# ZhehuiWu/MP-HSIR

Hardware: AMD Instinct MI355X
Metric: hsi_patches_per_sec_fwd_bwd (higher is better)
Workload: dtype bf16; 1 GPU; natural-scene MP_HSIR_Net(31,31,64,T=6) training step fwd+bwd+allreduce+AdamW, 64x64x31 patches, batch 32/GPU, dp1; global_batch=32, patch=64x64x31, parallelism=dp1, launch=hipGraph replay

## Files before the change

include/mphsir.h:

```cpp
#ifndef MPHSIR_H
#define MPHSIR_H
#include <stddef.h>
#include <stdint.h>

#ifdef __cplusplus
extern "C" {
#endif

#define MPHSIR_OK 0
#define MPHSIR_EINVAL (-1)
#define MPHSIR_ELAUNCH (-2)

#define MPHSIR_F32 0
#define MPHSIR_BF16 1
#define MPHSIR_F16 2

const char* mphsir_version(void);
const char* mphsir_last_error(void);
int mphsir_device_arch(char* buf, int n);

typedef struct mphsir_gemm_args {
    uint32_t struct_size;
    const void* X; int64_t ldx;
    const void* W; int64_t w_batch_stride; int64_t rows_per_batch;
// ... 129 lines not shown
    const void* W1; const float* b1; const void* W1T; const void* W2T;
    void* dX; void* XN; void* H; void* DPRE; float* part;
    int64_t M; int32_t C, HP;
    int32_t variant;
    const float* keep;
    int64_t rows_per_batch;
    int32_t hsplit;
    float* dxn_part;
} mphsir_mlp_bwd_args;
int mphsir_gated_mlp_bwd(const mphsir_mlp_bwd_args* a, int dtype, void* stream);

typedef struct mphsir_mlp_wgrad_args {
    uint32_t struct_size;
    const void* XN; const void* DM;
    const void* W1; const float* b1; const void* W2T;
    float* dW1p; float* dW2p; float* db1p; float* db2p;
    int64_t M; int32_t C, HP;
    int32_t ranges;
    int32_t chunks_per_wg;
} mphsir_mlp_wgrad_args;
int mphsir_gated_mlp_wgrad(const mphsir_mlp_wgrad_args* a, int dtype, void* stream);
int mphsir_gated_mlp_wgrad_fits(int32_t C, int32_t chunks_per_wg, int dtype);

int mphsir_combine_bwd(const void* dY, const void* SA, const float* gate, const float* keep, void* dOut, void* dSA,
                       float* dgate, int32_t B, int32_t H, int32_t W, int32_t C, int32_t shift, int dtype, void* stream);
typedef struct mphsir_win_attn_bwd_args {
    uint32_t struct_size;
    const void* X; const void* dSA; const float* dmu;
    const float* ln_w; const float* ln_b;
    const void* Wqkv; const float* bqkv; const float* rpb; const void* WprojT;
    void* dQKV; void* XNw; void* dSAt; float* drpb;
    int32_t B, H, W, C, heads, shift;
    int32_t head_split;
} mphsir_win_attn_bwd_args;
int mphsir_win_attn_bwd(const mphsir_win_attn_bwd_args* a, int dtype, void* stream);
int mphsir_win_attn_bwd_fits(int32_t C, int32_t heads, int dtype);
int mphsir_ln_bwd_win(const void* X, const void* dXNw, const void* dRes, const float* ln_w, void* dX, float* part,
                      int32_t B, int32_t H, int32_t W, int32_t C, int32_t shift, const float* ln_b, void* XN, int32_t linear,
                      int dtype, void* stream);

int mphsir_ln_bwd_win_dxn(const void* X, const void* dQKV, const void* WqkvT, const void* dRes, const void* dRes2, const float* ln_w, void* dX,
                          float* part, int32_t B, int32_t H, int32_t W, int32_t C, int32_t shift, int dtype, void* stream);
int mphsir_ln_bwd_win_dxn_fits(int32_t C, int dtype);
int mphsir_ln_bwd_tok_dxn(const void* X, const void* dY, const void* WT, const void* dRes, const float* ln_w, const float* ln_b, void* dX,
                          void* XN, float* part, int64_t M, int32_t C, int32_t K, int32_t x_f32, int dtype, void* stream);

int mphsir_layernorm_tok(const void* X, int x_dtype, const float* ln_w, const float* ln_b, void* Y, void* Xcopy, int y_dtype,
                         int64_t M, int32_t C, void* stream);

typedef struct mphsir_fold_bwd_args {
    uint32_t struct_size;
    const float* Gpart; const float* Spart; const float* temperature; const float* Wo; const float* dM;
    void* W2; float* dWo; float* dtemp;
    int32_t B, C, heads, nsplit;
    int32_t dM_nsplit;
    const void* DO; int64_t lddo; const void* V; int64_t ldv; int32_t N;
    int32_t w2_blocks;
} mphsir_fold_bwd_args;
int mphsir_spectral_fold_bwd(const mphsir_fold_bwd_args* a, int dtype, void* stream);
typedef struct mphsir_pg_bwd_args {
    uint32_t struct_size;
    const float* mu; const float* dgate;
    const float* Wprompt; const float* prompt_param; const float* Wq; const float* Wkv; const float* Wdown;
    const float* Wpproj; const float* bpproj; const float* Wup;
    float* dmu; void* L; void* R;
    int32_t nW, C, r, KL, KR;
    int32_t lr_bf16;
} mphsir_pg_bwd_args;
int mphsir_pg_gate_bwd(const mphsir_pg_bwd_args* a, void* stream);
// ... 241 lines not shown
```

mp-hsir_amd/_lib.py:

```python
import ctypes
import os

import torch

_HERE = os.path.dirname(os.path.abspath(__file__))
_PATH = os.path.join(_HERE, os.environ.get("MPHSIR_LIB_AB", "libmphsir.so"))
_lib = None
_is_emu = False

c_void_p, c_int64, c_int32, c_int, c_float_p = (ctypes.c_void_p, ctypes.c_int64, ctypes.c_int32, ctypes.c_int,
                                                ctypes.POINTER(ctypes.c_float))


class _Args(ctypes.Structure):

    def __init__(self, *args, **kw):
        super().__init__(*args, **kw)
        self.struct_size = ctypes.sizeof(self)


_SZ = [("struct_size", ctypes.c_uint32)]


class GemmArgs(_Args):
# ... 37 lines not shown
               [("T", c_void_p), ("ldt", c_int64), ("QK", c_void_p), ("ldqk", c_int64), ("row_segments", c_int32)]


class FoldArgs(_Args):
    _fields_ = _SZ + [("Gpart", c_void_p), ("Spart", c_void_p), ("temperature", c_void_p), ("Wo", c_void_p), ("M", c_void_p),
                ("MT", c_void_p)] + \
               [(n, c_int32) for n in ("B", "C", "heads", "nsplit")] + [("Gsum", c_void_p), ("Ssum", c_void_p)]


class GateArgs(_Args):
    _fields_ = _SZ + [("T", c_void_p), ("ldt", c_int64), ("w9", c_void_p), ("ldw", c_int64), ("U", c_void_p), ("ldu", c_int64)] + \
               [(n, c_int32) for n in ("B", "H", "W", "HP")]


class GdfnArgs(_Args):
    _fields_ = _SZ + [("X", c_void_p), ("ldx", c_int64), ("ln_w", c_void_p), ("ln_b", c_void_p), ("Win", c_void_p), ("w9", c_void_p),
                ("ldw", c_int64), ("Wout", c_void_p), ("Y", c_void_p), ("ldy", c_int64)] + \
               [(n, c_int32) for n in ("B", "H", "W", "D", "HP", "nsplit")] + [("T", c_void_p), ("ldt", c_int64)]


class MlpBwdArgs(_Args):
    _fields_ = _SZ + [(n, c_void_p) for n in ("X", "dY", "DM", "ln_w", "ln_b", "W1", "b1", "W1T", "W2T", "dX", "XN", "H", "DPRE", "part")] + \
               [("M", c_int64), ("C", c_int32), ("HP", c_int32), ("variant", c_int32), ("keep", c_void_p), ("rows_per_batch", c_int64),
                ("hsplit", c_int32), ("dxn_part", c_void_p)]


class MlpWgradArgs(_Args):
    _fields_ = _SZ + [(n, c_void_p) for n in ("XN", "DM", "W1", "b1", "W2T", "dW1p", "dW2p", "db1p", "db2p")] + \
               [("M", c_int64), ("C", c_int32), ("HP", c_int32), ("ranges", c_int32), ("chunks_per_wg", c_int32)]


class WinAttnBwdArgs(_Args):
    _fields_ = _SZ + [(n, c_void_p) for n in ("X", "dSA", "dmu", "ln_w", "ln_b", "Wqkv", "bqkv", "rpb", "WprojT", "dQKV", "XNw",
                                         "dSAt", "drpb")] + [(n, c_int32) for n in ("B", "H", "W", "C", "heads", "shift", "head_split")]


class FoldBwdArgs(_Args):
    _fields_ = _SZ + [(n, c_void_p) for n in ("Gpart", "Spart", "temperature", "Wo", "dM", "W2", "dWo", "dtemp")] + \
               [(n, c_int32) for n in ("B", "C", "heads", "nsplit", "dM_nsplit")] + \
               [("DO", c_void_p), ("lddo", c_int64), ("V", c_void_p), ("ldv", c_int64), ("N", c_int32), ("w2_blocks", c_int32)]


class PgBwdArgs(_Args):
    _fields_ = _SZ + [(n, c_void_p) for n in ("mu", "dgate", "Wprompt", "prompt_param", "Wq", "Wkv", "Wdown", "Wpproj", "bpproj", "Wup",
                                         "dmu", "L", "R")] + [(n, c_int32) for n in ("nW", "C", "r", "KL", "KR", "lr_bf16")]


class SpectralBwdArgs(_Args):
    _fields_ = _SZ + [("QK", c_void_p), ("ldqk", c_int64), ("DO", c_void_p), ("lddo", c_int64), ("T", c_void_p), ("ldt", c_int64),
                      ("W2", c_void_p), ("MbT", c_void_p), ("w9", c_void_p), ("ldw", c_int64), ("dT", c_void_p), ("lddt", c_int64),
                      ("part", c_void_p)] + [(n, c_int32) for n in ("B", "H", "W", "C", "heads", "nblk", "round_dall")]


class SceneGatherArgs(_Args):
    _fields_ = _SZ + [("scene", c_void_p), ("origins", c_void_p), ("tiles", c_void_p)] + [(n, c_int32) for n in ("n", "C", "H", "W", "th", "tw")]


class SceneBlendArgs(_Args):
    _fields_ = _SZ + [("tiles", c_void_p), ("oy", c_void_p), ("ox", c_void_p), ("scene", c_void_p)] + \
               [(n, c_int32) for n in ("ny", "nx", "C", "H", "W", "th", "tw", "ov", "clamp01")]


class SceneGatherD4Args(_Args):
    _fields_ = _SZ + [("scene", c_void_p), ("origins", c_void_p), ("tiles", c_void_p)] + \
               [(n, c_int32) for n in ("j0", "count", "n_tiles", "G", "modes_packed", "C", "H", "W", "th", "tw")]


# ... 53 lines not shown
    "mphsir_layernorm_tok": (c_int, [c_void_p, c_int, c_void_p, c_void_p, c_void_p, c_void_p, c_int, c_int64, c_int32, c_void_p]),
    "mphsir_win_attn_fwd": (c_int, [ctypes.POINTER(WinAttnArgs), c_int, c_void_p]),
    "mphsir_win_attn_hdp": (c_int, [c_int, c_int]),
    "mphsir_pg_gate_fwd": (c_int, [ctypes.POINTER(PgFwdArgs), c_void_p]),
    "mphsir_dwconv_gram": (c_int, [ctypes.POINTER(GramArgs), c_int, c_void_p]),
    "mphsir_dwconv_gram_keeps_qk": (c_int, [c_int32, c_int32, c_int]),
    "mphsir_qkv_dwconv_gram": (c_int, [ctypes.POINTER(FusedGramArgs), c_int, c_void_p]),
    "mphsir_qkv_dwconv_gram_fits": (c_int, [c_int32, c_int32, c_int32, c_int32, c_int]),
    "mphsir_qkv_dwconv_gram_rows_fits": (c_int, [c_int32, c_int32, c_int32, c_int32, c_int, c_int32]),
    "mphsir_debug": (c_int, [c_int, c_void_p]),
    "mphsir_dwconv3x3_wgrad_tiled": (c_int, [c_int32, c_int32, c_int32, c_int]),
    "mphsir_spectral_fold": (c_int, [ctypes.POINTER(FoldArgs), c_int, c_void_p]),
    "mphsir_dwconv_gate": (c_int, [ctypes.POINTER(GateArgs), c_int, c_void_p]),
    "mphsir_dwconv_gate_bwd": (c_int, [c_void_p, c_void_p, c_int64, c_void_p, c_void_p, c_void_p, c_int32, c_int32, c_int32, c_int32, c_int, c_void_p]),
    "mphsir_dwconv_gate_bwd_fits": (c_int, [c_int32, c_int32, c_int32, c_int]),
    "mphsir_gdfn_fused": (c_int, [ctypes.POINTER(GdfnArgs), c_int, c_void_p]),
    "mphsir_gdfn_fused_fits": (c_int, [c_int32, c_int32, c_int32, c_int32, c_int]),
    "mphsir_gdfn_fused_tile_width": (c_int, [c_int32]),
    "mphsir_dwconv3x3": (c_int, [c_void_p, c_int64, c_void_p, c_int64, c_void_p, c_int64, c_int32, c_int32, c_int32, c_int32,
                                 c_int32, c_int, c_void_p]),
    "mphsir_dwconv3x3_bwd": (c_int, [c_void_p, c_int64, c_void_p, c_int64, c_void_p, c_int64, c_void_p, c_int64, c_void_p, c_int32, c_int32, c_int32,
                                     c_int32, c_int32, c_int, c_void_p]),
    "mphsir_dwconv3x3_wgrad": (c_int, [c_void_p, c_int64, c_void_p, c_int64, c_void_p, c_int32, c_int32, c_int32, c_int32,
                                       c_int32, c_int, c_void_p]),
    "mphsir_flat_adamw": (c_int, [c_void_p, c_void_p, c_void_p, c_void_p, c_int64, ctypes.c_float, ctypes.c_float,
                                  ctypes.c_float, ctypes.c_float, ctypes.c_float, c_int32, ctypes.c_float, c_void_p, c_void_p]),
    "mphsir_grad_check": (c_int, [c_void_p, c_int64, c_void_p, c_void_p]),
    "mphsir_flat_adamw_scaled": (c_int, [c_void_p, c_void_p, c_void_p, c_void_p, c_int64, ctypes.c_float, ctypes.c_float, ctypes.c_float,
                                         ctypes.c_float, ctypes.c_float, ctypes.c_float, c_void_p, c_void_p, c_void_p]),
    "mphsir_scaler_update": (c_int, [c_void_p, ctypes.c_float, ctypes.c_float, c_int32, c_void_p]),
    "mphsir_combine_bwd": (c_int, [c_void_p] * 7 + [c_int32] * 5 + [c_int, c_void_p]),
    "mphsir_win_attn_bwd": (c_int, [ctypes.POINTER(WinAttnBwdArgs), c_int, c_void_p]),
    "mphsir_win_attn_bwd_fits": (c_int, [c_int32, c_int32, c_int]),
    "mphsir_ln_bwd_win": (c_int, [c_void_p] * 6 + [c_int32] * 5 + [c_void_p, c_void_p, c_int32, c_int, c_void_p]),
    "mphsir_ln_bwd_win_dxn": (c_int, [c_void_p] * 8 + [c_int32] * 5 + [c_int, c_void_p]),
    "mphsir_ln_bwd_win_dxn_fits": (c_int, [c_int32, c_int]),
    "mphsir_ln_bwd_tok_dxn": (c_int, [c_void_p] * 9 + [c_int64, c_int32, c_int32, c_int32, c_int, c_void_p]),
    "mphsir_gemm_tn": (c_int, [c_void_p, c_int64, c_int64, c_void_p, c_int64, c_int64, c_void_p, c_void_p, c_int64, c_int32, c_int32,
                               c_int32, c_int32, c_int32, c_int, c_void_p]),
    "mphsir_spectral_fold_bwd": (c_int, [ctypes.POINTER(FoldBwdArgs), c_int, c_void_p]),
    "mphsir_pg_gate_bwd": (c_int, [ctypes.POINTER(PgBwdArgs), c_void_p]),
    "mphsir_spectral_dqkv_bwd": (c_int, [ctypes.POINTER(SpectralBwdArgs), c_int, c_void_p]),
    "mphsir_spectral_dqkv_bwd_fits": (c_int, [c_int32, c_int32, c_int32, c_int32, c_int]),
    "mphsir_spectral_dqkv_bwd_slabs": (c_int, [c_int32, c_int32]),
    "mphsir_conv3x3_tok": (c_int, [c_void_p, c_int64, c_void_p, c_void_p, c_int64, c_int32, c_int32, c_int32, c_int32, c_int32,
                                   c_int, c_void_p]),
    "mphsir_conv3x3_wgrad": (c_int, [c_void_p, c_int64, c_void_p, c_int64, c_void_p, c_int32, c_int32, c_int32, c_int32, c_int32, c_int32, c_int32, c_int, c_void_p]),
    "mphsir_im2col3x3": (c_int, [c_void_p, c_int64, c_void_p, c_int32, c_int32, c_int32, c_int32, c_int, c_void_p]),
    "mphsir_gdfn_gate_bwd": (c_int, [c_void_p, c_void_p, c_void_p, c_void_p, c_int64, c_int32, c_int, c_void_p]),
    "mphsir_gated_mlp_bwd": (c_int, [ctypes.POINTER(MlpBwdArgs), c_int, c_void_p]),
    "mphsir_gated_mlp_wgrad": (c_int, [ctypes.POINTER(MlpWgradArgs), c_int, c_void_p]),
    "mphsir_gated_mlp_wgrad_fits": (c_int, [c_int32, c_int32, c_int]),
    "mphsir_gated_mlp_fwd": (c_int, [ctypes.POINTER(MlpArgs), c_int, c_void_p]),
    "mphsir_gated_mlp_fwd_fuses": (c_int, [c_int32, c_int64, c_int]),
    "mphsir_reduce_parts": (c_int, [ctypes.POINTER(ReduceSeg), c_int32, c_void_p]),
    "mphsir_gemm_tn_group": (c_int, [ctypes.POINTER(TnProblem), c_int32, c_int32, c_int, c_void_p]),
    "mphsir_pack_gather": (c_int, [c_void_p, c_void_p, c_void_p, c_int64, c_int, c_void_p]),
    "mphsir_multi_copy": (c_int, [c_void_p, c_int32, c_int64, c_void_p]),
    "mphsir_nchw_to_cl": (c_int, [c_void_p, c_void_p, c_int32, c_int32, c_int64, c_int32, c_int, c_void_p]),
    "mphsir_cl_to_nchw_add": (c_int, [c_void_p, c_int64, c_void_p, c_void_p, c_int32, c_int32, c_int64, c_int, c_void_p]),
    "mphsir_task_weights": (c_int, [c_void_p, c_void_p, c_int32, c_int32, c_int32, c_void_p]),
    "mphsir_mix_rows": (c_int, [c_void_p, c_void_p, c_void_p, c_int32, c_int32, c_int32, ctypes.c_float, c_int32, c_void_p]),
    "mphsir_scene_gather": (c_int, [ctypes.POINTER(SceneGatherArgs), c_void_p]),
    "mphsir_scene_blend": (c_int, [ctypes.POINTER(SceneBlendArgs), c_void_p]),
    "mphsir_scene_gather_d4": (c_int, [ctypes.POINTER(SceneGatherD4Args), c_void_p]),
    "mphsir_scene_fold_d4": (c_int, [ctypes.POINTER(SceneFoldD4Args), c_void_p]),
# ... 51 lines not shown
```

mp-hsir_amd/autograd_ops.py:

```python
from collections import namedtuple

import torch
import torch.nn.functional as F

from . import ops


class SkipGrad:

    def __init__(self):
        self.dz = None

    def take(self):
        dz, self.dz = self.dz, None
        return dz


Skip = namedtuple("Skip", "holder first last")


def _skip_put(skip, dz, needed):
    if not needed:
        return None
    if skip is not None and skip.last:
# ... 162 lines not shown

def _pgsstb_attn_forward(blk, k1, x, fuse=False):
    B, H, W, Cc = x.shape
    dt = x.dtype
    pk = blk.packed(dt)
    sp = blk.gobal_spectral_attn.packed(dt)
    heads, shift = blk.num_heads, blk.shift_size
    sa, mu, oattn = ops.win_attn_fwd(x, pk["ln1"][0], pk["ln1"][1], pk["wqkv"], pk["bqkv"], pk["rpb"], pk["wproj"],
                                     pk["bproj"], pk["pg"], heads, shift, save=True, gate=False)
    with ops.side_stream(sa, ops.SIDE_BRANCH) as br:
        gate = ops.pg_gate_fwd(mu, pk["pg"])
    sa2 = sa.reshape(-1, Cc)
    v, gp, spart, t, qk = _pass_a(sa2, sp["wqkv"], sp["w9"], B, H, W, Cc, heads, keep=True)
    Mb, MbT, gp, spart = ops.spectral_fold(gp, spart, sp["temp"], sp["wo"], dt, transposed=True)
    br.join()
    saved = _AttnSaved(x, sa, gate, mu, oattn, t, v, gp, spart, Mb, MbT, qk)
    if fuse:
        return None, saved
    y = ops.gemm_tok(v, Mb, epi=2, res=x.reshape(-1, Cc), sa=sa2, gate=gate, keep=k1, geom=(H, W, shift))
    return y.reshape(B, H, W, Cc), saved


def _pgsstb_attn_backward(blk, k1, saved, dy, extra=None):
    x, sa, gate, mu, oattn = saved.x, saved.sa, saved.gate, saved.mu, saved.oattn
    B, H, W, Cc = x.shape
    dt = x.dtype
    M = B * H * W
    heads, shift = blk.num_heads, blk.shift_size
    pk = blk.packed(dt)
    sp = blk.gobal_spectral_attn.packed(dt)
    dy = dy.contiguous()
    with ops.reduce_scope(leaf=True):
        f32_factors = dt == torch.float16 or mu.shape[0] <= 512
        d_out, d_sa, dgate = ops.combine_bwd(dy, sa, gate, k1, shift)
        with ops.side_stream(dy, ops.SIDE_BRANCH) as br:
            dmu, gpg = ops.pg_gate_bwd(mu, dgate, pk["pg"], factor_dtype=torch.float32 if f32_factors else dt)
        dt3, d_sdw, dtemp, dwo = channel_attention_bwd_self(
            d_out.reshape(M, Cc), saved.t.reshape(B, H, W, 3 * Cc), sp["w9"], saved.v, saved.gp, saved.spart, saved.MbT,
            blk.gobal_spectral_attn.temperature, blk.gobal_spectral_attn.project_out.weight, heads, qk=saved.qk)
        d_sa = ops.gemm_tok(dt3, sp["wqkvT"], epi=1, res=d_sa.reshape(M, Cc))
        d_sqkv = ops.gemm_tn(dt3, sa.reshape(M, Cc)).reshape(3 * Cc, Cc, 1, 1)
        dpg = tuple(gpg[k].reshape(getattr_path(blk.local_spectral_attn, k).shape) for k in _PG_KEYS)
        br.join()
        dqkv, xnw, dsat, drpb = ops.win_attn_bwd(x, d_sa.reshape(B, H, W, Cc), dmu, pk["ln1"][0], pk["ln1"][1], pk["wqkv"], pk["bqkv"],
                                                 pk["rpb"], pk["wprojT"], heads, shift)
        d_qkv_w, d_qkv_b = ops.gemm_tn(dqkv, xnw, colsum=True)
        dsat2 = dsat.reshape(M, Cc)
        d_proj_w, d_proj_b = ops.gemm_tn(dsat2, oattn.reshape(M, Cc), colsum=True)
        if ops.ln_bwd_win_dxn_fits(M, Cc, dt):
            dx, part = ops.ln_bwd_win_dxn(x, dqkv, pk["wqkvT"], dy, pk["ln1"][0], shift, dres2=None if extra is None else extra.contiguous())
        else:
            dx, part = ops.ln_bwd_win(x, ops.gemm_tok(dqkv, pk["wqkvT"]), dy, pk["ln1"][0], shift)
            if extra is not None:
                dx = dx + extra
        dln = ops.reduce_parts(part)
        drpb = ops.reduce_parts(drpb)
    return (dx, dln[0], dln[1], d_qkv_w, d_qkv_b, d_proj_w, d_proj_b, drpb,
            dtemp.reshape(heads, 1, 1), d_sqkv, d_sdw.reshape(3 * Cc, 1, 3, 3), dwo.reshape(Cc, Cc, 1, 1)) + tuple(dpg)


class _PgsstbAttn(torch.autograd.Function):

    @staticmethod
    def forward(ctx, blk, k1, skip, x, n1w, n1b, qkv_w, qkv_b, proj_w, proj_b, rpb, s_temp, s_qkv, s_dw, s_out, *pg):
        y, saved = _pgsstb_attn_forward(blk, k1, x)
        ctx.blk, ctx.k1, ctx.skip = blk, k1, skip
        ctx.save_for_backward(*saved)
        return y

    @staticmethod
    def backward(ctx, dy):
        return (None, None, None) + _pgsstb_attn_backward(ctx.blk, ctx.k1, _AttnSaved(*ctx.saved_tensors), dy, extra=_skip_take(ctx.skip))


_N_ATTN_PARAMS = 11 + len(_PG_KEYS)


class _Pgsstb(torch.autograd.Function):
# ... 458 lines not shown
```

mp-hsir_amd/csrc/block_bwd.hip:

```cpp
#include "mphsir_dev.h"
#include "mphsir_host.h"

namespace mphsir {

struct WinGeom {
    int B, H, W, shift;
};

__device__ __forceinline__ long win_pixel(const WinGeom& g, int blk, int t) {
    const int nwx = g.W >> 3, nW = (g.H >> 3) * nwx;
    const int b = blk / nW, wi = blk % nW, wy = wi / nwx, wx = wi % nwx;
    const int ys = wy * 8 + (t >> 3), xs = wx * 8 + (t & 7);
    return ((long)b * g.H + (ys + g.shift) % g.H) * g.W + (xs + g.shift) % g.W;
}

struct CombBwdDev {
    const void* dY; const void* SA; const float* gate; const float* keep;
    void* dOut;
    void* dSA;
    float* dgate;
    WinGeom g; int C;
};

template <class T>
__global__ __launch_bounds__(256) void combine_bwd_kernel(CombBwdDev a) {
    constexpr int VEC = Vec16<T>::N;
    __shared__ float red[256 * VEC];
    const int C = a.C, tid = threadIdx.x, nv = C / VEC;
    const int groups = 256 / nv < 64 ? 256 / nv : 64, grp = tid / nv, cv = tid % nv, c0 = cv * VEC;
    const int nW = (a.g.H >> 3) * (a.g.W >> 3), b = blockIdx.x / nW;
    const float kf = a.keep ? a.keep[b] : 1.f;
    const T* dY = reinterpret_cast<const T*>(a.dY);
    const T* SA = reinterpret_cast<const T*>(a.SA);
    T* dOut = reinterpret_cast<T*>(a.dOut);
    T* dSA = reinterpret_cast<T*>(a.dSA);
    const float* g = a.gate + (long)blockIdx.x * C;
    float acc[VEC];
    for (int e = 0; e < VEC; ++e) acc[e] = 0.f;
    if (grp < groups) {
        float gv[VEC];
        for (int e = 0; e < VEC; ++e) gv[e] = g[c0 + e];
        for (int t = grp; t < 64; t += groups) {
            const long p = win_pixel(a.g, blockIdx.x, t) * C + c0;
            const Vec16<T> dy = load16<T>(dY + p), sa = load16<T>(SA + p);
            Vec16<T> o, s;
            for (int e = 0; e < VEC; ++e) {
                const float d = to_f32(from_f32<T>(kf * dy.get(e)));
                o.set(e, d);
                s.set(e, d * gv[e]);
                acc[e] += d * sa.get(e);
            }
            if (a.keep && dOut) store16<T>(dOut + p, o);
            store16<T>(dSA + p, s);
        }
        for (int e = 0; e < VEC; ++e) red[grp * C + c0 + e] = acc[e];
    }
    __syncthreads();
    for (int c = tid; c < C; c += 256) {
        float sum = 0.f;
        for (int gi = 0; gi < groups; ++gi) sum += red[gi * C + c];
        a.dgate[(long)blockIdx.x * C + c] = sum;
    }
}

struct WinBwdDev {
    const void* X; const void* dSA; const float* dmu;
    const float* ln_w; const float* ln_b;
    const void* Wqkv; const float* bqkv; const float* rpb;
    const void* WprojT;
    void* dQKV;
    void* XNw;
    void* dSAt;
    float* drpb;
    WinGeom g;
    int hsplit;
};

template <class T, int C, int HD, bool XL> struct WinBwdCfg {
    static constexpr int PAD = LDS_PAD_BYTES / sizeof(T);
    static constexpr int HEADS = C / HD;
    static constexpr int KC = ElemTraits<T>::KCHUNK;
    static constexpr int HDP = (HD + KC - 1) / KC * KC;
    static constexpr int LDX = C + PAD;
    static constexpr int LDQ = HDP + PAD;
    static constexpr int LDT = 64 + PAD;
    static constexpr bool ALIAS = HDP >= 64;
    static constexpr size_t XS = XL ? 64 * LDX : 0, QS = 64 * LDQ, SS = 64 * LDT;
    static constexpr size_t T_ELEMS = XS + 4 * QS + (ALIAS ? 1 : 2) * SS;
    static constexpr size_t BYTES = T_ELEMS * sizeof(T) + (225 + 64) * 4;
    static constexpr bool FITS = BYTES <= 160 * 1024;
    static constexpr int LDWS = C + PAD;
    static constexpr int SR = (size_t)HD * LDWS <= SS ? HD : (HD % 32 == 0 && (size_t)32 * LDWS <= SS) ? 32 : ((size_t)16 * LDWS <= SS ? 16 : 0);
    static constexpr bool STAGE = SR > 0;
};

template <class T, int C, int HD> struct WinBwdPick {
    static constexpr bool XL = WinBwdCfg<T, C, HD, true>::BYTES <= 80 * 1024;
};

template <class T, int C, int HD, bool XL, bool XR = false>
__global__ __launch_bounds__(256, XR ? 3 : 1) void win_attn_bwd_kernel(WinBwdDev a) {
    typedef ElemTraits<T> TR;
    typedef typename TR::frag_t frag_t;
    typedef WinBwdCfg<T, C, HD, XL> CF;
    static_assert(!XR || (!XL && CF::HDP == HD && CF::STAGE && 64 * (C + CF::PAD) <= 4 * CF::QS), "XR: no X tile, no K padding, staged weights");
    constexpr int VEC = Vec16<T>::N;
    constexpr int TPW = HD / 16;
    HIP_DYNAMIC_SHARED(f32x4, smem_v)
    T* Xs = reinterpret_cast<T*>(smem_v);
    T* Qr = Xs + CF::XS;
    T* Kr = Qr + CF::QS;
    T* Vr = Kr + CF::QS;
    T* Or = Vr + CF::QS;
    T* dS = Or + CF::QS;
    T* Ps = CF::ALIAS ? Vr : dS + CF::SS;
    float* rpbs = reinterpret_cast<float*>(Xs + CF::T_ELEMS);
    int* reg = reinterpret_cast<int*>(rpbs + 225);

    const int tid = threadIdx.x, lane = tid & 63, wv = wave_id_uniform();
    const T* X = reinterpret_cast<const T*>(a.X);
    const T* dSA = reinterpret_cast<const T*>(a.dSA);
    const long row0 = (long)blockIdx.x * 64;
    const T* Xg = reinterpret_cast<const T*>(a.XNw) + row0 * C;
    const T* Dg = reinterpret_cast<const T*>(a.dSAt) + row0 * C;

    {
        constexpr int NV = C / VEC, VPT = NV / 4;
        const int t = tid >> 2, q = tid & 3;
        const long pix = win_pixel(a.g, blockIdx.x, t);
        const T* row = X + pix * C;
        Vec16<T> xv[VPT];
        float s = 0.f;
#pragma unroll
        for (int i = 0; i < VPT; ++i) {
            xv[i] = load16<T>(row + (q + 4 * i) * VEC);
            for (int e = 0; e < VEC; ++e) s += xv[i].get(e);
        }
        s += __shfl_xor(s, 1);
        s += __shfl_xor(s, 2);
        const float mean = s / (float)C;
        float d2 = 0.f;
#pragma unroll
        for (int i = 0; i < VPT; ++i)
            for (int e = 0; e < VEC; ++e) { float d = xv[i].get(e) - mean; d2 += d * d; }
        d2 += __shfl_xor(d2, 1);
        d2 += __shfl_xor(d2, 2);
        const float rstd = rsqrtf(d2 / (float)C + 1e-5f);
        T* xnw = reinterpret_cast<T*>(a.XNw) + (row0 + t) * C;
        T* dst = reinterpret_cast<T*>(a.dSAt) + (row0 + t) * C;
        const float* dmu = a.dmu + (long)blockIdx.x * C;
#pragma unroll
        for (int i = 0; i < VPT; ++i) {
            const int c0 = (q + 4 * i) * VEC;
            Vec16<T> o;
            for (int e = 0; e < VEC; ++e) o.set(e, (xv[i].get(e) - mean) * rstd * a.ln_w[c0 + e] + a.ln_b[c0 + e]);
            if (XL) store16<T>(Xs + t * CF::LDX + c0, o);
            if (XR) store16<T>(Qr + t * CF::LDX + c0, o);
            store16<T>(xnw + c0, o);
            Vec16<T> d = load16<T>(dSA + pix * C + c0);
            for (int e = 0; e < VEC; ++e) d.set(e, d.get(e) + dmu[c0 + e] * (1.0f / 64.0f));
            store16<T>(dst + c0, d);
        }
        if (tid < 64) {
            const int nwx = a.g.W >> 3, nW = (a.g.H >> 3) * nwx, wi = blockIdx.x % nW;
            const int ys = (wi / nwx) * 8 + (tid >> 3), xs = (wi % nwx) * 8 + (tid & 7);
            const int ry = (ys >= a.g.H - 8) + (ys >= a.g.H - 4), rx = (xs >= a.g.W - 8) + (xs >= a.g.W - 4);
            reg[tid] = a.g.shift ? 3 * ry + rx : 0;
        }
        if (CF::HDP != HD)
            for (int i = tid; i < 4 * 64 * (CF::HDP - HD); i += 256) {
                const int rr = i / (CF::HDP - HD), cc = HD + i % (CF::HDP - HD);
                Qr[rr * CF::LDQ + cc] = from_f32<T>(0.f);
            }
    }

    const T* Wqkv = reinterpret_cast<const T*>(a.Wqkv);
    const T* WpT = reinterpret_cast<const T*>(a.WprojT);
    T* dQKV = reinterpret_cast<T*>(a.dQKV);
    const float scale = rsqrtf((float)HD);

    constexpr int WSR = CF::STAGE ? CF::SR : 16;
    constexpr int WVT = WSR * (C / VEC), NWV = (WVT + 255) / 256;
    Vec16<T> wpre[NWV];
    auto wload = [&](int h, int sub) __attribute__((always_inline)) {
        const int which = sub / (HD / WSR), r0 = (sub % (HD / WSR)) * WSR;
        const T* Wsrc = (which < 3 ? Wqkv + (long)(which * C) * C : WpT) + (long)(h * HD + r0) * C;
#pragma unroll
        for (int i = 0; i < NWV; ++i) {
            const int idx = tid + 256 * i;
            if (idx < WVT) wpre[i] = load16<T>(Wsrc + (long)(idx / (C / VEC)) * C + (idx % (C / VEC)) * VEC);
        }
    };
    auto wstore = [&]() __attribute__((always_inline)) {
#pragma unroll
// ... 345 lines not shown

template <class T, int C, int HD>
static int launch_win_bwd(const WinBwdDev& d, hipStream_t s) {
    if constexpr (sizeof(T) == 2 && (C == 64 || (C == 128 && HD == 64)) && (HD == 32 || HD == 64)) return launch_win_bwd_xr<T, C, HD>(d, s);
    constexpr bool PICK = WinBwdPick<T, C, HD>::XL;
    constexpr int ov = -1;
    if constexpr (WinBwdCfg<T, C, HD, true>::FITS) {
        if (ov == 1 || (ov < 0 && PICK)) return launch_win_bwd_xl<T, C, HD, true>(d, s);
    }
    return launch_win_bwd_xl<T, C, HD, false>(d, s);
}

#define MPHSIR_WINB_SHAPES(X) X(32, 32) X(64, 32) X(64, 64) X(128, 32) X(128, 64) X(256, 32) X(96, 48) X(192, 48) X(192, 96) X(384, 48)

template <class T>
static int dispatch_win_bwd(const WinBwdDev& d, int C, int HD, hipStream_t s) {
#define MPHSIR_WINB_CASE(c, hd) if (C == c && HD == hd) return launch_win_bwd<T, c, hd>(d, s);
    MPHSIR_WINB_SHAPES(MPHSIR_WINB_CASE)
#undef MPHSIR_WINB_CASE
    set_error("win_attn_bwd: (C=%d, head_dim=%d) not instantiated", C, HD);
    return MPHSIR_EINVAL;
}

static bool geom_ok(int B, int H, int W, int shift) {
    return B > 0 && H > 0 && W > 0 && H % 8 == 0 && W % 8 == 0 && (shift == 0 || shift == 4);
}

}

extern "C" int mphsir_combine_bwd(const void* dY, const void* SA, const float* gate, const float* keep, void* dOut, void* dSA,
                                  float* dgate, int32_t B, int32_t H, int32_t W, int32_t C, int32_t shift, int dtype, void* stream) {
    using namespace mphsir;
    clear_error();
    MPHSIR_REQUIRE(dY && SA && gate && dSA && dgate, "combine_bwd: null pointer");
    MPHSIR_REQUIRE(MPHSIR_DTYPE_OK(dtype), "combine_bwd: dtype %d unsupported", dtype);
    MPHSIR_REQUIRE(geom_ok(B, H, W, shift) && C > 0 && C % 8 == 0, "combine_bwd: bad geometry");
    MPHSIR_REQUIRE(aligned16(dY) && aligned16(SA) && aligned16(dSA) && (!dOut || aligned16(dOut)), "combine_bwd: 16-byte alignment required");
    CombBwdDev d{dY, SA, gate, keep, dOut, dSA, dgate, WinGeom{B, H, W, shift}, C};
    const int nblk = B * (H / 8) * (W / 8);
    hipStream_t s = reinterpret_cast<hipStream_t>(stream);
    if (dtype == MPHSIR_F32)
        MPHSIR_LAUNCH(MPHSIR_K_COMBINE_BWD, (combine_bwd_kernel<float>), dim3(nblk), dim3(256), 0, s, d);
    else if (dtype == MPHSIR_BF16)
        MPHSIR_LAUNCH(MPHSIR_K_COMBINE_BWD, (combine_bwd_kernel<bf16_t>), dim3(nblk), dim3(256), 0, s, d);
    else
        MPHSIR_LAUNCH(MPHSIR_K_COMBINE_BWD, (combine_bwd_kernel<f16_t>), dim3(nblk), dim3(256), 0, s, d);
    return MPHSIR_OK;
}

extern "C" int mphsir_win_attn_bwd(const mphsir_win_attn_bwd_args* a, int dtype, void* stream) {
    using namespace mphsir;
    clear_error();
    MPHSIR_CHECK_ARGS(a, "win_attn_bwd");
    MPHSIR_REQUIRE(a && a->X && a->dSA && a->dmu && a->ln_w && a->ln_b && a->Wqkv && a->bqkv && a->rpb && a->WprojT && a->dQKV &&
                       a->XNw && a->dSAt && a->drpb, "win_attn_bwd: null pointer");
    MPHSIR_REQUIRE(MPHSIR_DTYPE_OK(dtype), "win_attn_bwd: dtype %d unsupported", dtype);
    MPHSIR_REQUIRE(geom_ok(a->B, a->H, a->W, a->shift) && a->heads > 0 && a->C % a->heads == 0, "win_attn_bwd: bad geometry");
    int hsplit = 1;
    const long nwin = (long)a->B * (a->H / 8) * (a->W / 8);
    while (nwin * hsplit < 512 && a->heads % (2 * hsplit) == 0) hsplit *= 2;
    if (a->head_split > 0) {
        MPHSIR_REQUIRE(a->heads % a->head_split == 0, "win_attn_bwd: head_split=%d must divide heads=%d", a->head_split, a->heads);
        hsplit = a->head_split;
    }
    WinBwdDev d{a->X, a->dSA, a->dmu, a->ln_w, a->ln_b, a->Wqkv, a->bqkv, a->rpb, a->WprojT, a->dQKV, a->XNw, a->dSAt, a->drpb,
                WinGeom{a->B, a->H, a->W, a->shift}, hsplit};
    hipStream_t s = reinterpret_cast<hipStream_t>(stream);
    return MPHSIR_DISPATCH_T(dtype, (dispatch_win_bwd<T_>(d, a->C, a->C / a->heads, s)));
}

extern "C" int mphsir_win_attn_bwd_fits(int32_t C, int32_t heads, int dtype) {
    if (heads <= 0 || C % heads != 0 || !MPHSIR_DTYPE_OK(dtype)) return 0;
    const int hd = C / heads;
#define MPHSIR_WINB_CASE(c, h_) if (C == c && hd == h_) return 1;
    MPHSIR_WINB_SHAPES(MPHSIR_WINB_CASE)
#undef MPHSIR_WINB_CASE
    return 0;
}

extern "C" int mphsir_ln_bwd_win(const void* X, const void* dXNw, const void* dRes, const float* ln_w, void* dX, float* part,
                                 int32_t B, int32_t H, int32_t W, int32_t C, int32_t shift, const float* ln_b, void* XN, int32_t linear,
                                 int dtype, void* stream) {
    using namespace mphsir;
    clear_error();
    MPHSIR_REQUIRE(X && dXNw && dRes && ln_w && dX && part, "ln_bwd_win: null pointer");
    MPHSIR_REQUIRE(MPHSIR_DTYPE_OK(dtype), "ln_bwd_win: dtype %d unsupported", dtype);
    MPHSIR_REQUIRE(geom_ok(B, H, W, shift) && C > 0 && C % 32 == 0 && C <= 512, "ln_bwd_win: bad geometry");
    MPHSIR_REQUIRE(aligned16(X) && aligned16(dXNw) && aligned16(dRes) && aligned16(dX), "ln_bwd_win: 16-byte alignment required");
    MPHSIR_REQUIRE(!XN || ln_b, "ln_bwd_win: XN output needs ln_b");
    LnBwdDev d{X, dXNw, dRes, ln_w, dX, part, WinGeom{B, H, W, shift}, C, ln_b, XN, linear};
    const size_t shmem = (64 * (size_t)(C + 1) + 256 + 3) * sizeof(float);
    const int nblk = B * (H / 8) * (W / 8);
    hipStream_t s = reinterpret_cast<hipStream_t>(stream);
    const int vec = 16 / dtype_size(dtype), vpt = (C / vec + 3) / 4;
#define MPHSIR_LNB(MV)                                                                                                   \
    return MPHSIR_DISPATCH_T(dtype, ([&]() -> int {                                                                      \
        allow_big_lds(ln_bwd_win_kernel<T_, MV>, shmem);                                                                 \
        MPHSIR_LAUNCH(MPHSIR_K_LN_BWD_WIN, (ln_bwd_win_kernel<T_, MV>), dim3(nblk), dim3(256), shmem, s, d);             \
        return MPHSIR_OK;                                                                                                \
    }()))
    if (vpt <= 4) { MPHSIR_LNB(4); }
    if (vpt <= 8) { MPHSIR_LNB(8); }
    if (vpt <= 12) { MPHSIR_LNB(12); }
    if (vpt <= 16) { MPHSIR_LNB(16); }
#undef MPHSIR_LNB
    if (dtype == MPHSIR_F32 && vpt <= 32) {
        allow_big_lds(ln_bwd_win_kernel<float, 32>, shmem);
        MPHSIR_LAUNCH(MPHSIR_K_LN_BWD_WIN, (ln_bwd_win_kernel<float, 32>), dim3(nblk), dim3(256), shmem, s, d);
        return MPHSIR_OK;
    }
// ... 4 lines not shown
```

mp-hsir_amd/ops.py:

```python
import ctypes
import os
import weakref

import torch

from . import _lib

_DT = {torch.float32: 0, torch.bfloat16: 1, torch.float16: 2}
_HALF = (torch.bfloat16, torch.float16)

ACCOUNT = None


def _acct(name, flops, nbytes):
    if ACCOUNT is not None:
        a = ACCOUNT.setdefault(name, [0, 0.0, 0.0])
        a[0] += 1
        a[1] += flops
        a[2] += nbytes


def _p(t):
    return None if t is None else ctypes.c_void_p(t.data_ptr())

# ... 1289 lines not shown
    nch, R = mlp_wgrad_plan(M, C, HP, xn.dtype, nch, ranges)
    dev = xn.device
    dW1p = torch.empty((R, 2 * HP, C), dtype=torch.float32, device=dev)
    dW2p = torch.empty((R, C, HP), dtype=torch.float32, device=dev)
    db1p = torch.empty((R, 1, 2 * HP), dtype=torch.float32, device=dev)
    db2p = torch.empty((R, C), dtype=torch.float32, device=dev)
    a = _lib.MlpWgradArgs()
    a.XN, a.DM, a.W1, a.b1, a.W2T = _p(xn), _p(dm), _p(W1), _p(b1), _p(W2T)
    a.dW1p, a.dW2p, a.db1p, a.db2p = _p(dW1p), _p(dW2p), _p(db1p), _p(db2p)
    a.M, a.C, a.HP, a.ranges, a.chunks_per_wg = M, C, HP, R, nch
    dt = _DT[xn.dtype]

    def run():
        _lib.check(lib.mphsir_gated_mlp_wgrad(ctypes.byref(a), dt, _stream(xn)), "gated_mlp_wgrad")

    if _SCOPE is not None:
        _SCOPE.calls.append(dict(run=run, keep=(xn, dm, W1, b1, W2T, dW1p, dW2p, db1p, db2p, a)))
    else:
        run()
    _acct("gated_mlp_wgrad", 12.0 * M * C * HP, 2.0 * M * C * xn.element_size())
    _acct("gated_mlp_wgrad:partials", 0.0, (dW1p.numel() + dW2p.numel()) * 4.0)
    dW1 = torch.empty((2 * hid, C), dtype=torch.float32, device=dev)
    db1 = torch.empty((1, 2 * hid), dtype=torch.float32, device=dev)
    dW2 = torch.empty((C, hid), dtype=torch.float32, device=dev)
    reduce_block(dW1p, 0, hid, 0, C, dW1[:hid])
    reduce_block(dW1p, HP, hid, 0, C, dW1[hid:])
    reduce_block(db1p, 0, 1, 0, hid, db1[:, :hid])
    reduce_block(db1p, 0, 1, HP, hid, db1[:, hid:])
    reduce_block(dW2p, 0, C, 0, hid, dW2)
    db2 = reduce_parts(db2p)
    return dW1, db1[0], dW2, db2


def combine_bwd(dy, sa, gate, keep, shift):
    lib = _lib.load()
    _check(dy, sa, gate, keep)
    B, H, W, C = dy.shape
    assert dy.is_contiguous() and sa.is_contiguous()
    d_out = torch.empty_like(dy) if keep is not None else dy
    d_sa = torch.empty_like(dy)
    dgate = torch.empty_like(gate)
    _lib.check(lib.mphsir_combine_bwd(_p(dy), _p(sa), _p(gate), _p(keep), _p(d_out) if keep is not None else None, _p(d_sa),
                                      _p(dgate), B, H, W, C, shift, _DT[dy.dtype], _stream(dy)), "combine_bwd")
    _acct("combine_bwd", 4.0 * dy.numel(), 4.0 * dy.numel() * dy.element_size())
    return d_out, d_sa, dgate


def win_attn_bwd_fits(C, heads, dtype):
    return bool(_lib.load().mphsir_win_attn_bwd_fits(C, heads, _DT[dtype]))


def win_attn_bwd(x, dsa, dmu, ln_w, ln_b, Wqkv, bqkv, rpb, WprojT, heads, shift, head_split=0):
    lib = _lib.load()
    _check(x, dsa, dmu, Wqkv, WprojT)
    B, H, W, C = x.shape
    M = B * H * W
    assert x.is_contiguous() and dsa.is_contiguous() and WprojT.shape == (C, C)
    dqkv = torch.empty((M, 3 * C), dtype=x.dtype, device=x.device)
    xnw = torch.empty((M, C), dtype=x.dtype, device=x.device)
    dsat = torch.empty_like(x)
    drpb = torch.empty((M // 64, 225, heads), dtype=torch.float32, device=x.device)
    a = _lib.WinAttnBwdArgs()
    a.X, a.dSA, a.dmu, a.ln_w, a.ln_b = _p(x), _p(dsa), _p(dmu), _p(ln_w), _p(ln_b)
    a.Wqkv, a.bqkv, a.rpb, a.WprojT = _p(Wqkv), _p(bqkv), _p(rpb), _p(WprojT)
    a.dQKV, a.XNw, a.dSAt, a.drpb = _p(dqkv), _p(xnw), _p(dsat), _p(drpb)
    a.B, a.H, a.W, a.C, a.heads, a.shift, a.head_split = B, H, W, C, heads, shift, head_split
    _lib.check(lib.mphsir_win_attn_bwd(ctypes.byref(a), _DT[x.dtype], _stream(x)), "win_attn_bwd")
    _acct("win_attn_bwd", M * (8.0 * C * C + 10.0 * 64 * C), 7.0 * M * C * x.element_size())
    return dqkv, xnw, dsat, drpb


def ln_bwd_win(x, dxn_w, dres, ln_w, shift):
    lib = _lib.load()
    _check(x, dxn_w, dres, ln_w)
    B, H, W, C = x.shape
    assert x.is_contiguous() and dxn_w.is_contiguous() and dres.is_contiguous()
    dx = torch.empty_like(x)
    part = torch.empty((B * H * W // 64, 2, C), dtype=torch.float32, device=x.device)
    _lib.check(lib.mphsir_ln_bwd_win(_p(x), _p(dxn_w), _p(dres), _p(ln_w), _p(dx), _p(part), B, H, W, C, shift, None, None, 0,
                                     _DT[x.dtype], _stream(x)), "ln_bwd_win")
    _acct("ln_bwd_win", 10.0 * x.numel(), 4.0 * x.numel() * x.element_size())
    return dx, part


LN_BWD_DXN = os.environ.get("MPHSIR_LN_BWD_DXN", "1") == "1"
LN_BWD_DXN_MAX_ROWS = int(os.environ.get("MPHSIR_LN_BWD_DXN_ROWS", "0"))


def ln_bwd_win_dxn_fits(M, C, dtype):
    return (LN_BWD_DXN and dtype in _HALF and (LN_BWD_DXN_MAX_ROWS == 0 or M <= LN_BWD_DXN_MAX_ROWS)
            and bool(_lib.load().mphsir_ln_bwd_win_dxn_fits(C, _DT[dtype])))


def ln_bwd_win_dxn(x, dqkv, wqkvT, dres, ln_w, shift, dres2=None):
    lib = _lib.load()
    _check(x, dqkv, wqkvT, dres, ln_w, dres2)
    B, H, W, C = x.shape
    assert x.is_contiguous() and dqkv.is_contiguous() and dres.is_contiguous() and wqkvT.is_contiguous()
    assert dqkv.shape == (B * H * W, 3 * C) and wqkvT.shape == (C, 3 * C) and wqkvT.dtype == x.dtype
    assert dres2 is None or (dres2.is_contiguous() and dres2.shape == x.shape and dres2.dtype == x.dtype)
    dx = torch.empty_like(x)
# ... 291 lines not shown
```

Baseline: 1719 patches/s.

## Fuse spectral-branch d_sa GEMM into window-attention backward kernel

The window-attention backward kernel can now build d_sa itself: it computes dT3·WsT with MFMA, staging weight chunks through LDS, and adds d_out*gate plus dmu/64 before its main work. Combine_bwd then skips writing d_sa, and the separate gemm_tok launch with its residual epilogue goes away. This removes one launch and a full write and read of the M×C d_sa tensor. In exchange the attention kernel carries an extra serial GEMM prologue per window, and the path is only used when head_split is 1.

New measurement: 1738 patches/s, median of 6. 1.01x the previous value.

```diff
diff --git a/include/mphsir.h b/include/mphsir.h
--- a/include/mphsir.h
+++ b/include/mphsir.h
@@ -185,9 +185,15 @@
     void* dQKV; void* XNw; void* dSAt; float* drpb;
     int32_t B, H, W, C, heads, shift;
     int32_t head_split;
+    const void* dT3;
+    const void* WsT;
+    const void* dOut;
+    const float* gate;
 } mphsir_win_attn_bwd_args;
 int mphsir_win_attn_bwd(const mphsir_win_attn_bwd_args* a, int dtype, void* stream);
 int mphsir_win_attn_bwd_fits(int32_t C, int32_t heads, int dtype);
+int mphsir_win_attn_bwd_dsa_fits(int32_t C, int32_t heads, int dtype);
+int mphsir_win_attn_bwd_head_split(int32_t B, int32_t H, int32_t W, int32_t heads);
 int mphsir_ln_bwd_win(const void* X, const void* dXNw, const void* dRes, const float* ln_w, void* dX, float* part,
                       int32_t B, int32_t H, int32_t W, int32_t C, int32_t shift, const float* ln_b, void* XN, int32_t linear,
                       int dtype, void* stream);
diff --git a/mp-hsir_amd/_lib.py b/mp-hsir_amd/_lib.py
--- a/mp-hsir_amd/_lib.py
+++ b/mp-hsir_amd/_lib.py
@@ -93,7 +93,8 @@
 
 class WinAttnBwdArgs(_Args):
     _fields_ = _SZ + [(n, c_void_p) for n in ("X", "dSA", "dmu", "ln_w", "ln_b", "Wqkv", "bqkv", "rpb", "WprojT", "dQKV", "XNw",
-                                         "dSAt", "drpb")] + [(n, c_int32) for n in ("B", "H", "W", "C", "heads", "shift", "head_split")]
+                                         "dSAt", "drpb")] + [(n, c_int32) for n in ("B", "H", "W", "C", "heads", "shift", "head_split")] + \
+               [(n, c_void_p) for n in ("dT3", "WsT", "dOut", "gate")]
 
 
 class FoldBwdArgs(_Args):
@@ -213,6 +214,8 @@
     "mphsir_combine_bwd": (c_int, [c_void_p] * 7 + [c_int32] * 5 + [c_int, c_void_p]),
     "mphsir_win_attn_bwd": (c_int, [ctypes.POINTER(WinAttnBwdArgs), c_int, c_void_p]),
     "mphsir_win_attn_bwd_fits": (c_int, [c_int32, c_int32, c_int]),
+    "mphsir_win_attn_bwd_dsa_fits": (c_int, [c_int32, c_int32, c_int]),
+    "mphsir_win_attn_bwd_head_split": (c_int, [c_int32] * 4),
     "mphsir_ln_bwd_win": (c_int, [c_void_p] * 6 + [c_int32] * 5 + [c_void_p, c_void_p, c_int32, c_int, c_void_p]),
     "mphsir_ln_bwd_win_dxn": (c_int, [c_void_p] * 8 + [c_int32] * 5 + [c_int, c_void_p]),
     "mphsir_ln_bwd_win_dxn_fits": (c_int, [c_int32, c_int]),
diff --git a/mp-hsir_amd/autograd_ops.py b/mp-hsir_amd/autograd_ops.py
--- a/mp-hsir_amd/autograd_ops.py
+++ b/mp-hsir_amd/autograd_ops.py
@@ -218,18 +218,23 @@
     dy = dy.contiguous()
     with ops.reduce_scope(leaf=True):
         f32_factors = dt == torch.float16 or mu.shape[0] <= 512
-        d_out, d_sa, dgate = ops.combine_bwd(dy, sa, gate, k1, shift)
+        own_dsa = ops.win_attn_bwd_dsa_fits(Cc, heads, dt) and ops.win_attn_bwd_dsa_pays(B, H, W, heads)
+        d_out, d_sa, dgate = ops.combine_bwd(dy, sa, gate, k1, shift, want_dsa=not own_dsa)
         with ops.side_stream(dy, ops.SIDE_BRANCH) as br:
             dmu, gpg = ops.pg_gate_bwd(mu, dgate, pk["pg"], factor_dtype=torch.float32 if f32_factors else dt)
         dt3, d_sdw, dtemp, dwo = channel_attention_bwd_self(
             d_out.reshape(M, Cc), saved.t.reshape(B, H, W, 3 * Cc), sp["w9"], saved.v, saved.gp, saved.spart, saved.MbT,
             blk.gobal_spectral_attn.temperature, blk.gobal_spectral_attn.project_out.weight, heads, qk=saved.qk)
-        d_sa = ops.gemm_tok(dt3, sp["wqkvT"], epi=1, res=d_sa.reshape(M, Cc))
+        if own_dsa:
+            branch = dict(dt3=dt3, wsT=sp["wqkvT"], d_out=d_out.reshape(M, Cc), gate=gate)
+        else:
+            branch = None
+            d_sa = ops.gemm_tok(dt3, sp["wqkvT"], epi=1, res=d_sa.reshape(M, Cc)).reshape(B, H, W, Cc)
         d_sqkv = ops.gemm_tn(dt3, sa.reshape(M, Cc)).reshape(3 * Cc, Cc, 1, 1)
         dpg = tuple(gpg[k].reshape(getattr_path(blk.local_spectral_attn, k).shape) for k in _PG_KEYS)
         br.join()
-        dqkv, xnw, dsat, drpb = ops.win_attn_bwd(x, d_sa.reshape(B, H, W, Cc), dmu, pk["ln1"][0], pk["ln1"][1], pk["wqkv"], pk["bqkv"],
-                                                 pk["rpb"], pk["wprojT"], heads, shift)
+        dqkv, xnw, dsat, drpb = ops.win_attn_bwd(x, d_sa, dmu, pk["ln1"][0], pk["ln1"][1], pk["wqkv"], pk["bqkv"],
+                                                 pk["rpb"], pk["wprojT"], heads, shift, branch=branch)
         d_qkv_w, d_qkv_b = ops.gemm_tn(dqkv, xnw, colsum=True)
         dsat2 = dsat.reshape(M, Cc)
         d_proj_w, d_proj_b = ops.gemm_tn(dsat2, oattn.reshape(M, Cc), colsum=True)
diff --git a/mp-hsir_amd/csrc/block_bwd.hip b/mp-hsir_amd/csrc/block_bwd.hip
--- a/mp-hsir_amd/csrc/block_bwd.hip
+++ b/mp-hsir_amd/csrc/block_bwd.hip
@@ -51,7 +51,7 @@
                 acc[e] += d * sa.get(e);
             }
             if (a.keep && dOut) store16<T>(dOut + p, o);
-            store16<T>(dSA + p, s);
+            if (dSA) store16<T>(dSA + p, s);
         }
         for (int e = 0; e < VEC; ++e) red[grp * C + c0 + e] = acc[e];
     }
@@ -74,6 +74,20 @@
     float* drpb;
     WinGeom g;
     int hsplit;
+    const void* dT3;
+    const void* WsT;
+    const void* dOut;
+    const float* gate;
+};
+
+template <class T, int C> struct WinBwdDsa {
+    static constexpr bool OK = sizeof(T) == 2 && (C == 64 || C == 128 || C == 256);
+    static constexpr int NB = C / 16, K = 3 * C, NKC = K / 32;
+    static constexpr int KGC = C <= 128 ? 3 : 2;
+    static constexpr int NGRP = NKC / KGC;
+    static constexpr int LDW = 32 * KGC + LDS_PAD_BYTES / (int)sizeof(T);
+    static constexpr int NWV = (C * KGC * 4 + 255) / 256;
+    static constexpr size_t BYTES = (size_t)C * LDW * sizeof(T);
 };
 
 template <class T, int C, int HD, bool XL> struct WinBwdCfg {
@@ -124,6 +138,67 @@
     const T* Xg = reinterpret_cast<const T*>(a.XNw) + row0 * C;
     const T* Dg = reinterpret_cast<const T*>(a.dSAt) + row0 * C;
 
+    bool own_dsa = false;
+    if constexpr (WinBwdDsa<T, C>::OK) {
+        typedef WinBwdDsa<T, C> DG;
+        static_assert(DG::BYTES <= CF::BYTES && DG::NKC % DG::KGC == 0, "the weight stage lies inside the kernel's LDS plan");
+        own_dsa = a.dT3 != nullptr;
+        if (own_dsa) {
+            T* Ws = reinterpret_cast<T*>(smem_v);
+            const T* WsT = reinterpret_cast<const T*>(a.WsT);
+            const int tok = wv * 16 + (lane & 15);
+            const long pix = win_pixel(a.g, blockIdx.x, tok);
+            const T* drow = reinterpret_cast<const T*>(a.dT3) + pix * DG::K + 8 * (lane >> 4);
+            Vec16<T> wreg[DG::NWV];
+            auto gload = [&](int g) __attribute__((always_inline)) {
+#pragma unroll
+                for (int i = 0; i < DG::NWV; ++i) {
+                    const int idx = tid + 256 * i;
+                    if (idx < C * DG::KGC * 4)
+                        wreg[i] = load16<T>(WsT + (long)(idx / (DG::KGC * 4)) * DG::K + g * 32 * DG::KGC + (idx % (DG::KGC * 4)) * VEC);
+                }
+            };
+            auto gstore = [&]() __attribute__((always_inline)) {
+#pragma unroll
+                for (int i = 0; i < DG::NWV; ++i) {
+                    const int idx = tid + 256 * i;
+                    if (idx < C * DG::KGC * 4) store16<T>(Ws + (idx / (DG::KGC * 4)) * DG::LDW + (idx % (DG::KGC * 4)) * VEC, wreg[i]);
+                }
+            };
+            f32x4 acc[DG::NB];
+#pragma unroll
+            for (int nb = 0; nb < DG::NB; ++nb) acc[nb] = f32x4{0.f, 0.f, 0.f, 0.f};
+            gload(0);
+#pragma unroll 1
+            for (int g = 0; g < DG::NGRP; ++g) {
+                frag_t df[DG::KGC];
+#pragma unroll
+                for (int kc = 0; kc < DG::KGC; ++kc) df[kc] = *reinterpret_cast<const frag_t*>(drow + (g * DG::KGC + kc) * 32);
+                if (g > 0) __syncthreads();
+                gstore();
+                __syncthreads();
+                if (g + 1 < DG::NGRP) gload(g + 1);
+#pragma unroll
+                for (int kc = 0; kc < DG::KGC; ++kc)
+#pragma unroll
+                    for (int nb = 0; nb < DG::NB; ++nb) mma(acc[nb], load_frag<T>(Ws, DG::LDW, nb * 16, kc * 32), df[kc]);
+            }
+            const int cr = (lane >> 4) * 4;
+            const T* orow = reinterpret_cast<const T*>(a.dOut) + pix * C + cr;
+            const float* grow = a.gate + (long)blockIdx.x * C + cr;
+            const float* mrow = a.dmu + (long)blockIdx.x * C + cr;
+            T* dst = reinterpret_cast<T*>(a.dSAt) + (row0 + tok) * C + cr;
+#pragma unroll
+            for (int nb = 0; nb < DG::NB; ++nb) {
+                const f32x4 o = load4<T>(orow + nb * 16);
+                const f32x4 gt = *reinterpret_cast<const f32x4*>(grow + nb * 16), mu = *reinterpret_cast<const f32x4*>(mrow + nb * 16);
+                f32x4 tot;
+                for (int r = 0; r < 4; ++r) tot[r] = acc[nb][r] + o[r] * gt[r] + mu[r] * (1.0f / 64.0f);
+                store4<T>(dst + nb * 16, tot);
+            }
+            __syncthreads();
+        }
+    }
     {
         constexpr int NV = C / VEC, VPT = NV / 4;
         const int t = tid >> 2, q = tid & 3;
@@ -157,9 +232,11 @@
             if (XL) store16<T>(Xs + t * CF::LDX + c0, o);
             if (XR) store16<T>(Qr + t * CF::LDX + c0, o);
             store16<T>(xnw + c0, o);
-            Vec16<T> d = load16<T>(dSA + pix * C + c0);
-            for (int e = 0; e < VEC; ++e) d.set(e, d.get(e) + dmu[c0 + e] * (1.0f / 64.0f));
-            store16<T>(dst + c0, d);
+            if (!own_dsa) {
+                Vec16<T> d = load16<T>(dSA + pix * C + c0);
+                for (int e = 0; e < VEC; ++e) d.set(e, d.get(e) + dmu[c0 + e] * (1.0f / 64.0f));
+                store16<T>(dst + c0, d);
+            }
         }
         if (tid < 64) {
             const int nwx = a.g.W >> 3, nW = (a.g.H >> 3) * nwx, wi = blockIdx.x % nW;
@@ -571,10 +648,10 @@
                                   float* dgate, int32_t B, int32_t H, int32_t W, int32_t C, int32_t shift, int dtype, void* stream) {
     using namespace mphsir;
     clear_error();
-    MPHSIR_REQUIRE(dY && SA && gate && dSA && dgate, "combine_bwd: null pointer");
+    MPHSIR_REQUIRE(dY && SA && gate && dgate, "combine_bwd: null pointer");
     MPHSIR_REQUIRE(MPHSIR_DTYPE_OK(dtype), "combine_bwd: dtype %d unsupported", dtype);
     MPHSIR_REQUIRE(geom_ok(B, H, W, shift) && C > 0 && C % 8 == 0, "combine_bwd: bad geometry");
-    MPHSIR_REQUIRE(aligned16(dY) && aligned16(SA) && aligned16(dSA) && (!dOut || aligned16(dOut)), "combine_bwd: 16-byte alignment required");
+    MPHSIR_REQUIRE(aligned16(dY) && aligned16(SA) && (!dSA || aligned16(dSA)) && (!dOut || aligned16(dOut)), "combine_bwd: 16-byte alignment required");
     CombBwdDev d{dY, SA, gate, keep, dOut, dSA, dgate, WinGeom{B, H, W, shift}, C};
     const int nblk = B * (H / 8) * (W / 8);
     hipStream_t s = reinterpret_cast<hipStream_t>(stream);
@@ -587,23 +664,37 @@
     return MPHSIR_OK;
 }
 
+extern "C" int mphsir_win_attn_bwd_head_split(int32_t B, int32_t H, int32_t W, int32_t heads) {
+    if (B <= 0 || H < 8 || W < 8 || heads <= 0) return 1;
+    int hsplit = 1;
+    const long nwin = (long)B * (H / 8) * (W / 8);
+    while (nwin * hsplit < 512 && heads % (2 * hsplit) == 0) hsplit *= 2;
+    return hsplit;
+}
+
 extern "C" int mphsir_win_attn_bwd(const mphsir_win_attn_bwd_args* a, int dtype, void* stream) {
     using namespace mphsir;
     clear_error();
     MPHSIR_CHECK_ARGS(a, "win_attn_bwd");
-    MPHSIR_REQUIRE(a && a->X && a->dSA && a->dmu && a->ln_w && a->ln_b && a->Wqkv && a->bqkv && a->rpb && a->WprojT && a->dQKV &&
+    const bool own_dsa = a->dT3 || a->WsT || a->dOut || a->gate;
+    MPHSIR_REQUIRE(a->X && (a->dSA || own_dsa) && a->dmu && a->ln_w && a->ln_b && a->Wqkv && a->bqkv && a->rpb && a->WprojT && a->dQKV &&
                        a->XNw && a->dSAt && a->drpb, "win_attn_bwd: null pointer");
     MPHSIR_REQUIRE(MPHSIR_DTYPE_OK(dtype), "win_attn_bwd: dtype %d unsupported", dtype);
     MPHSIR_REQUIRE(geom_ok(a->B, a->H, a->W, a->shift) && a->heads > 0 && a->C % a->heads == 0, "win_attn_bwd: bad geometry");
-    int hsplit = 1;
-    const long nwin = (long)a->B * (a->H / 8) * (a->W / 8);
-    while (nwin * hsplit < 512 && a->heads % (2 * hsplit) == 0) hsplit *= 2;
+    if (own_dsa) {
+        MPHSIR_REQUIRE(a->dT3 && a->WsT && a->dOut && a->gate, "win_attn_bwd: dT3, WsT, dOut and gate go together (all four or none)");
+        MPHSIR_REQUIRE(mphsir_win_attn_bwd_dsa_fits(a->C, a->heads, dtype),
+                       "win_attn_bwd: (C=%d, heads=%d, dtype=%d) does not form d_sa itself (ask mphsir_win_attn_bwd_dsa_fits)", a->C, a->heads, dtype);
+        MPHSIR_REQUIRE(aligned16(a->dT3) && aligned16(a->WsT) && aligned16(a->dOut) && aligned16(a->gate) && aligned16(a->dmu) && aligned16(a->dSAt),
+                       "win_attn_bwd: 16-byte alignment required");
+    }
+    int hsplit = mphsir_win_attn_bwd_head_split(a->B, a->H, a->W, a->heads);
     if (a->head_split > 0) {
         MPHSIR_REQUIRE(a->heads % a->head_split == 0, "win_attn_bwd: head_split=%d must divide heads=%d", a->head_split, a->heads);
         hsplit = a->head_split;
     }
     WinBwdDev d{a->X, a->dSA, a->dmu, a->ln_w, a->ln_b, a->Wqkv, a->bqkv, a->rpb, a->WprojT, a->dQKV, a->XNw, a->dSAt, a->drpb,
-                WinGeom{a->B, a->H, a->W, a->shift}, hsplit};
+                WinGeom{a->B, a->H, a->W, a->shift}, hsplit, a->dT3, a->WsT, a->dOut, a->gate};
     hipStream_t s = reinterpret_cast<hipStream_t>(stream);
     return MPHSIR_DISPATCH_T(dtype, (dispatch_win_bwd<T_>(d, a->C, a->C / a->heads, s)));
 }
@@ -615,6 +706,10 @@
     MPHSIR_WINB_SHAPES(MPHSIR_WINB_CASE)
 #undef MPHSIR_WINB_CASE
     return 0;
+}
+
+extern "C" int mphsir_win_attn_bwd_dsa_fits(int32_t C, int32_t heads, int dtype) {
+    return ((dtype == MPHSIR_BF16 || dtype == MPHSIR_F16) && (C == 64 || C == 128 || C == 256) && mphsir_win_attn_bwd_fits(C, heads, dtype)) ? 1 : 0;
 }
 
 extern "C" int mphsir_ln_bwd_win(const void* X, const void* dXNw, const void* dRes, const float* ln_w, void* dX, float* part,
diff --git a/mp-hsir_amd/ops.py b/mp-hsir_amd/ops.py
--- a/mp-hsir_amd/ops.py
+++ b/mp-hsir_amd/ops.py
@@ -1345,17 +1345,18 @@
     return dW1, db1[0], dW2, db2
 
 
-def combine_bwd(dy, sa, gate, keep, shift):
+def combine_bwd(dy, sa, gate, keep, shift, want_dsa=True):
     lib = _lib.load()
     _check(dy, sa, gate, keep)
     B, H, W, C = dy.shape
     assert dy.is_contiguous() and sa.is_contiguous()
     d_out = torch.empty_like(dy) if keep is not None else dy
-    d_sa = torch.empty_like(dy)
+    d_sa = torch.empty_like(dy) if want_dsa else None
     dgate = torch.empty_like(gate)
     _lib.check(lib.mphsir_combine_bwd(_p(dy), _p(sa), _p(gate), _p(keep), _p(d_out) if keep is not None else None, _p(d_sa),
                                       _p(dgate), B, H, W, C, shift, _DT[dy.dtype], _stream(dy)), "combine_bwd")
-    _acct("combine_bwd", 4.0 * dy.numel(), 4.0 * dy.numel() * dy.element_size())
+    passes = 2.0 + (keep is not None) + bool(want_dsa)
+    _acct("combine_bwd", passes * dy.numel(), passes * dy.numel() * dy.element_size())
     return d_out, d_sa, dgate
 
 
@@ -1363,12 +1364,34 @@
     return bool(_lib.load().mphsir_win_attn_bwd_fits(C, heads, _DT[dtype]))
 
 
-def win_attn_bwd(x, dsa, dmu, ln_w, ln_b, Wqkv, bqkv, rpb, WprojT, heads, shift, head_split=0):
+BRANCH_BWD_FUSED = os.environ.get("MPHSIR_BRANCH_BWD_FUSED", "1") == "1"
+
+
+def win_attn_bwd_dsa_fits(C, heads, dtype):
+    return BRANCH_BWD_FUSED and dtype in _HALF and bool(_lib.load().mphsir_win_attn_bwd_dsa_fits(C, heads, _DT[dtype]))
+
+
+BRANCH_BWD_SPLIT_HEADS_TOO = False
+
+
+def win_attn_bwd_dsa_pays(B, H, W, heads):
+    return BRANCH_BWD_SPLIT_HEADS_TOO or _lib.load().mphsir_win_attn_bwd_head_split(B, H, W, heads) == 1
+
+
+def win_attn_bwd(x, dsa, dmu, ln_w, ln_b, Wqkv, bqkv, rpb, WprojT, heads, shift, head_split=0, branch=None):
     lib = _lib.load()
     _check(x, dsa, dmu, Wqkv, WprojT)
     B, H, W, C = x.shape
     M = B * H * W
-    assert x.is_contiguous() and dsa.is_contiguous() and WprojT.shape == (C, C)
+    assert x.is_contiguous() and WprojT.shape == (C, C)
+    if branch is None:
+        assert dsa.is_contiguous()
+    else:
+        dt3, wsT, d_out, gate = branch["dt3"], branch["wsT"], branch["d_out"], branch["gate"]
+        _check(x, dt3, wsT, d_out, gate)
+        assert dsa is None and dt3.is_contiguous() and d_out.is_contiguous() and wsT.is_contiguous() and gate.is_contiguous()
+        assert dt3.shape == (M, 3 * C) and wsT.shape == (C, 3 * C) and d_out.numel() == M * C and gate.shape == (M // 64, C)
+        assert dt3.dtype == wsT.dtype == d_out.dtype == x.dtype and gate.dtype == dmu.dtype == torch.float32
     dqkv = torch.empty((M, 3 * C), dtype=x.dtype, device=x.device)
     xnw = torch.empty((M, C), dtype=x.dtype, device=x.device)
     dsat = torch.empty_like(x)
@@ -1378,8 +1401,10 @@
     a.Wqkv, a.bqkv, a.rpb, a.WprojT = _p(Wqkv), _p(bqkv), _p(rpb), _p(WprojT)
     a.dQKV, a.XNw, a.dSAt, a.drpb = _p(dqkv), _p(xnw), _p(dsat), _p(drpb)
     a.B, a.H, a.W, a.C, a.heads, a.shift, a.head_split = B, H, W, C, heads, shift, head_split
+    if branch is not None:
+        a.dT3, a.WsT, a.dOut, a.gate = _p(dt3), _p(wsT), _p(d_out), _p(gate)
     _lib.check(lib.mphsir_win_attn_bwd(ctypes.byref(a), _DT[x.dtype], _stream(x)), "win_attn_bwd")
-    _acct("win_attn_bwd", M * (8.0 * C * C + 10.0 * 64 * C), 7.0 * M * C * x.element_size())
+    _acct("win_attn_bwd", M * ((8.0 if branch is None else 14.0) * C * C + 10.0 * 64 * C), (7.0 if branch is None else 10.0) * M * C * x.element_size())
     return dqkv, xnw, dsat, drpb
 
 
```
